# TaceoLabs/co-snarks

Measured on NVIDIA H100. Metric: co-Groth16 proofs/sec (BN254, 2^20 constraints); MSM Mscalar/s, higher is better.
Workload: dtype u32x8 (256-bit Montgomery, integer)

## Files before the change

### co_snarks_b200/csrc/cs_curve.cuh

```cuda
#pragma once
#include "cs_field.cuh"

namespace cs {

template <class P>
struct Fp2 {
  typedef Fp<P> F;
  static constexpr int N = 2 * P::N;
  F c0, c1;
  static CS_D Fp2 zero() { Fp2 r; r.c0 = F::zero(); r.c1 = F::zero(); return r; }
  static CS_D Fp2 one() { Fp2 r; r.c0 = F::one(); r.c1 = F::zero(); return r; }
  CS_D bool is_zero() const { return c0.is_zero() && c1.is_zero(); }
  CS_D bool operator==(const Fp2& b) const { return c0 == b.c0 && c1 == b.c1; }
  CS_D bool operator!=(const Fp2& b) const { return !(*this == b); }
  friend CS_D Fp2 operator+(const Fp2& a, const Fp2& b) { Fp2 r; r.c0 = a.c0 + b.c0; r.c1 = a.c1 + b.c1; return r; }
  friend CS_D Fp2 operator-(const Fp2& a, const Fp2& b) { Fp2 r; r.c0 = a.c0 - b.c0; r.c1 = a.c1 - b.c1; return r; }
  friend CS_D Fp2 operator*(const Fp2& a, const Fp2& b) { return mul_ool(a, b); }
  static CS_DN Fp2 mul_ool(Fp2 a, Fp2 b) {
    F v0 = F::mul_inline(a.c0, b.c0), v1 = F::mul_inline(a.c1, b.c1);
    F v2 = F::mul_inline(a.c0 + a.c1, b.c0 + b.c1);
    Fp2 r;
    r.c1 = v2 - v0 - v1;
    r.c0 = v0 - v1;
    return r;
  }
  CS_D Fp2 sqr() const { return sqr_ool(*this); }
  static CS_DN Fp2 sqr_ool(Fp2 a) {
    Fp2 r;
    F t = F::mul_inline(a.c0, a.c1);
    r.c0 = F::mul_inline(a.c0 + a.c1, a.c0 - a.c1);
    r.c1 = t + t;
    return r;
  }
  CS_D Fp2 neg() const { Fp2 r; r.c0 = c0.neg(); r.c1 = c1.neg(); return r; }
  CS_D Fp2 dbl() const { Fp2 r; r.c0 = c0.dbl(); r.c1 = c1.dbl(); return r; }
  CS_D Fp2 inverse() const {
    F n = (c0.sqr() + c1.sqr()).inverse();
    Fp2 r;
    r.c0 = c0 * n;
    r.c1 = (c1 * n).neg();
    return r;
  }
};

template <class P>
CS_D Fp<P> mul_sub(const Fp<P>& a, const Fp<P>& b, const Fp<P>& c, const Fp<P>& d) { return Fp<P>::dot2(a, b, c.neg(), d); }
template <class P>
CS_D Fp2<P> mul_sub(const Fp2<P>& a, const Fp2<P>& b, const Fp2<P>& c, const Fp2<P>& d) { return a * b - c * d; }

template <class F>
struct Affine {
  F x, y;
  CS_D bool is_inf() const { return x.is_zero() && y.is_zero(); }
  static CS_D Affine inf() { Affine r; r.x = F::zero(); r.y = F::zero(); return r; }
};

template <class F>
struct Xyzz {
  F x, y, zz, zzz;
  CS_D bool is_inf() const { return zz.is_zero(); }
  static CS_D Xyzz inf() {
    Xyzz r;
    r.x = F::zero(); r.y = F::zero(); r.zz = F::zero(); r.zzz = F::zero();
    return r;
  }
  static CS_D Xyzz from_affine(const Affine<F>& p) {
    if (p.is_inf()) return inf();
    Xyzz r;
    r.x = p.x; r.y = p.y; r.zz = F::one(); r.zzz = F::one();
    return r;
  }
};

template <class F>
CS_DN Xyzz<F> dbl_affine(const Affine<F>& p) {
  Xyzz<F> r;
  if (p.y.is_zero()) return Xyzz<F>::inf();
  F U = p.y.dbl();
  F V = U.sqr();
  F W = U * V;
  F S = p.x * V;
  F X2 = p.x.sqr();
  F M = X2.dbl() + X2;
  r.x = M.sqr() - S.dbl();
  r.y = mul_sub(M, S - r.x, W, p.y);
  r.zz = V;
  r.zzz = W;
  return r;
}

template <class F>
CS_DN Xyzz<F> dbl_xyzz(const Xyzz<F>& p) {
  if (p.is_inf() || p.y.is_zero()) return Xyzz<F>::inf();
  Xyzz<F> r;
  F U = p.y.dbl();
  F V = U.sqr();
  F W = U * V;
  F S = p.x * V;
  F X2 = p.x.sqr();
  F M = X2.dbl() + X2;
  r.x = M.sqr() - S.dbl();
  r.y = mul_sub(M, S - r.x, W, p.y);
  r.zz = V * p.zz;
  r.zzz = W * p.zzz;
  return r;
}

template <class F>
CS_D void madd(Xyzz<F>& acc, const Affine<F>& p_in, bool negate) {
  if (p_in.is_inf()) return;
  Affine<F> p = p_in;
  if (negate) p.y = p.y.neg();
  if (acc.is_inf()) {
    acc.x = p.x; acc.y = p.y; acc.zz = F::one(); acc.zzz = F::one();
    return;
  }
  F U2 = p.x * acc.zz;
  F S2 = p.y * acc.zzz;
  F Pp = U2 - acc.x;
  F R = S2 - acc.y;
  if (Pp.is_zero()) {
    if (R.is_zero()) acc = dbl_affine(p);
    else acc = Xyzz<F>::inf();
    return;
  }
  F PP = Pp.sqr();
  F PPP = Pp * PP;
  F Q = acc.x * PP;
  F X3 = R.sqr() - PPP - Q.dbl();
  acc.y = mul_sub(R, Q - X3, acc.y, PPP);
  acc.x = X3;
  acc.zz = acc.zz * PP;
  acc.zzz = acc.zzz * PPP;
}

template <class F>
CS_D void padd(Xyzz<F>& acc, const Xyzz<F>& q) {
  if (q.is_inf()) return;
  if (acc.is_inf()) { acc = q; return; }
  F U1 = acc.x * q.zz;
  F U2 = q.x * acc.zz;
  F S1 = acc.y * q.zzz;
  F S2 = q.y * acc.zzz;
  F Pp = U2 - U1;
  F R = S2 - S1;
  if (Pp.is_zero()) {
    if (R.is_zero()) acc = dbl_xyzz(acc);
    else acc = Xyzz<F>::inf();
    return;
  }
  F PP = Pp.sqr();
  F PPP = Pp * PP;
  F Q = U1 * PP;
  F X3 = R.sqr() - PPP - Q.dbl();
  acc.y = mul_sub(R, Q - X3, S1, PPP);
  acc.x = X3;
  acc.zz = acc.zz * q.zz * PP;
  acc.zzz = acc.zzz * q.zzz * PPP;
}

template <class P>
CS_D Fp<P> shfl_down(const Fp<P>& a, unsigned delta) {
  Fp<P> r;
#if defined(CS_EMU)
  cs::emu::shfl_bytes(&a, &r, sizeof(r), 1, delta);
  return r;
#endif
  CS_UNROLL
  for (int i = 0; i < P::N; i++) r.l[i] = __shfl_down_sync(0xffffffffu, a.l[i], delta);
  return r;
}
template <class P>
CS_D Fp2<P> shfl_down(const Fp2<P>& a, unsigned delta) {
  Fp2<P> r;
  r.c0 = shfl_down(a.c0, delta);
  r.c1 = shfl_down(a.c1, delta);
  return r;
}
template <class F>
CS_D Xyzz<F> shfl_down(const Xyzz<F>& p, unsigned delta) {
  Xyzz<F> r;
#if defined(CS_EMU)
  cs::emu::shfl_bytes(&p, &r, sizeof(r), 1, delta);
  return r;
#endif
  r.x = shfl_down(p.x, delta); r.y = shfl_down(p.y, delta);
  r.zz = shfl_down(p.zz, delta); r.zzz = shfl_down(p.zzz, delta);
  return r;
}

template <class F>
CS_DN Affine<F> to_affine(const Xyzz<F>& p) {
  if (p.is_inf()) return Affine<F>::inf();
  F zi = p.zzz.inverse();
  F zzi = (zi * p.zz).sqr();
  Affine<F> r;
  r.x = p.x * zzi;
  r.y = p.y * zi;
  return r;
}

}
```

### co_snarks_b200/csrc/cs_field.cuh

```cuda
#pragma once
#include "cs_prims.cuh"

namespace cs {

template <int N>
CS_D void mul_n(uint32_t* acc, const uint32_t* a, uint32_t bi) {
  CS_UNROLL
  for (int j = 0; j < N; j += 2) {
    acc[j] = mul_lo(a[j], bi);
    acc[j + 1] = mul_hi(a[j], bi);
  }
}

template <int N>
CS_D void cmad_n(uint32_t* acc, const uint32_t* a, uint32_t bi) {
  acc[0] = mad_lo_cc(a[0], bi, acc[0]);
  acc[1] = madc_hi_cc(a[0], bi, acc[1]);
  CS_UNROLL
  for (int j = 2; j < N; j += 2) {
    acc[j] = madc_lo_cc(a[j], bi, acc[j]);
    acc[j + 1] = madc_hi_cc(a[j], bi, acc[j + 1]);
  }
}

template <int N>
CS_D void madc_n_rshift(uint32_t* odd, const uint32_t* a, uint32_t bi) {
  CS_UNROLL
  for (int j = 0; j < N - 2; j += 2) {
    odd[j] = madc_lo_cc(a[j], bi, odd[j + 2]);
    odd[j + 1] = madc_hi_cc(a[j], bi, odd[j + 3]);
  }
  odd[N - 2] = madc_lo_cc(a[N - 2], bi, 0);
  odd[N - 1] = madc_hi(a[N - 2], bi, 0);
}

template <class P, bool FIRST>
CS_D void mad_n_redc(uint32_t* X, uint32_t* Y, const uint32_t* a, uint32_t bi) {
  constexpr int N = P::N;
  if (FIRST) {
    mul_n<N>(Y, a + 1, bi);
    mul_n<N>(X, a, bi);
  } else {
    X[0] = add_cc(X[0], Y[1]);
    madc_n_rshift<N>(Y, a + 1, bi);
    cmad_n<N>(X, a, bi);
    Y[N - 1] = addc(Y[N - 1], 0);
  }
  uint32_t mi = mul_lo(X[0], P::M0);
  uint32_t mod[N];
  CS_UNROLL
  for (int i = 0; i < N; i++) mod[i] = P::mod(i);
  cmad_n<N>(Y, mod + 1, mi);
  cmad_n<N>(X, mod, mi);
  Y[N - 1] = addc(Y[N - 1], 0);
}

template <class P>
struct Fp {
  static constexpr int N = P::N;
  uint32_t l[N];

  static CS_D Fp zero() { Fp r; CS_UNROLL for (int i = 0; i < N; i++) r.l[i] = 0; return r; }
  static CS_D Fp one() { Fp r; CS_UNROLL for (int i = 0; i < N; i++) r.l[i] = P::one(i); return r; }
  static CS_D Fp r2() { Fp r; CS_UNROLL for (int i = 0; i < N; i++) r.l[i] = P::r2(i); return r; }

  CS_D bool is_zero() const {
    uint32_t o = 0;
    CS_UNROLL
    for (int i = 0; i < N; i++) o |= l[i];
    return o == 0;
  }
  CS_D bool operator==(const Fp& b) const {
    uint32_t o = 0;
    CS_UNROLL
    for (int i = 0; i < N; i++) o |= l[i] ^ b.l[i];
    return o == 0;
  }
  CS_D bool operator!=(const Fp& b) const { return !(*this == b); }

  CS_D void final_sub() {
    uint32_t t[N];
    t[0] = sub_cc(l[0], P::mod(0));
    CS_UNROLL
    for (int i = 1; i < N; i++) t[i] = subc_cc(l[i], P::mod(i));
    uint32_t borrow = subc(0, 0);
    CS_UNROLL
    for (int i = 0; i < N; i++) l[i] = borrow ? l[i] : t[i];
  }

  friend CS_D Fp operator+(const Fp& a, const Fp& b) {
    Fp r;
    r.l[0] = add_cc(a.l[0], b.l[0]);
    CS_UNROLL
    for (int i = 1; i < N; i++) r.l[i] = addc_cc(a.l[i], b.l[i]);
    r.final_sub();
    return r;
  }
  friend CS_D Fp operator-(const Fp& a, const Fp& b) {
    Fp r;
    r.l[0] = sub_cc(a.l[0], b.l[0]);
    CS_UNROLL
    for (int i = 1; i < N; i++) r.l[i] = subc_cc(a.l[i], b.l[i]);
    uint32_t borrow = subc(0, 0);
    r.l[0] = add_cc(r.l[0], borrow & P::mod(0));
    CS_UNROLL
    for (int i = 1; i < N; i++) r.l[i] = addc_cc(r.l[i], borrow & P::mod(i));
    return r;
  }
  CS_D Fp neg() const { return is_zero() ? *this : (zero() - *this); }
  CS_D Fp dbl() const { return *this + *this; }

  friend CS_D Fp operator*(const Fp& a, const Fp& b) { return mul_ool(a, b); }
  static CS_DN Fp mul_ool(Fp a, Fp b) { return mul_inline(a, b); }
  static CS_D Fp mul_inline(const Fp& a, const Fp& b) {
    uint32_t even[N], odd[N];
    mad_n_redc<P, true>(even, odd, a.l, b.l[0]);
    mad_n_redc<P, false>(odd, even, a.l, b.l[1]);
    CS_UNROLL
    for (int i = 2; i < N; i += 2) {
      mad_n_redc<P, false>(even, odd, a.l, b.l[i]);
      mad_n_redc<P, false>(odd, even, a.l, b.l[i + 1]);
    }
    Fp r;
    r.l[0] = add_cc(even[0], odd[1]);
    CS_UNROLL
    for (int i = 1; i < N - 1; i++) r.l[i] = addc_cc(even[i], odd[i + 1]);
    r.l[N - 1] = addc(even[N - 1], 0);
    r.final_sub();
    return r;
  }
  CS_D Fp sqr() const { return sqr_ool(*this); }
  static CS_DN Fp sqr_ool(Fp a) {
    uint32_t c0 = 0, c1 = 0, c2 = 0;
    uint32_t m[N];
    Fp r;
    CS_UNROLL
    for (int k = 0; k < 2 * N - 1; k++) {
      uint32_t t0 = 0, t1 = 0, t2 = 0;
      CS_UNROLL
      for (int i = 0; i < N; i++) {
        int j = k - i;
        if (j > i && j < N) {
          t0 = mad_lo_cc(a.l[i], a.l[j], t0);
          t1 = madc_hi_cc(a.l[i], a.l[j], t1);
          t2 = addc(t2, 0);
        }
      }
      t2 = (t2 << 1) | (t1 >> 31);
      t1 = (t1 << 1) | (t0 >> 31);
      t0 = t0 << 1;
      c0 = add_cc(c0, t0);
      c1 = addc_cc(c1, t1);
      c2 = addc(c2, t2);
      if ((k & 1) == 0) {
        c0 = mad_lo_cc(a.l[k / 2], a.l[k / 2], c0);
        c1 = madc_hi_cc(a.l[k / 2], a.l[k / 2], c1);
        c2 = addc(c2, 0);
      }
      CS_UNROLL
      for (int i = 0; i < N; i++) {
        int j = k - i;
        if (i < k && i < N && j >= 0 && j < N && (k < N ? i < k : true)) {
          if (k < N || i >= k - N + 1) {
            c0 = mad_lo_cc(m[i], P::mod(j), c0);
            c1 = madc_hi_cc(m[i], P::mod(j), c1);
            c2 = addc(c2, 0);
          }
        }
      }
      if (k < N) {
        m[k] = mul_lo(c0, P::M0);
        c0 = mad_lo_cc(m[k], P::mod(0), c0);
        c1 = madc_hi_cc(m[k], P::mod(0), c1);
        c2 = addc(c2, 0);
      } else {
        r.l[k - N] = c0;
      }
      c0 = c1; c1 = c2; c2 = 0;
    }
    r.l[N - 1] = c0;
    r.final_sub();
    return r;
  }

  static CS_D Fp dot2(const Fp& a, const Fp& b, const Fp& c, const Fp& d) { return dot2_ool(a, b, c, d); }
  static CS_DN Fp dot2_ool(Fp a, Fp b, Fp c, Fp d) {
    uint32_t c0 = 0, c1 = 0, c2 = 0;
    uint32_t m[N];
    Fp r;
    CS_UNROLL
    for (int k = 0; k < 2 * N - 1; k++) {
      CS_UNROLL
      for (int i = 0; i < N; i++) {
        const int j = k - i;
        if (j >= 0 && j < N) {
          c0 = mad_lo_cc(a.l[i], b.l[j], c0);
          c1 = madc_hi_cc(a.l[i], b.l[j], c1);
          c2 = addc(c2, 0);
          c0 = mad_lo_cc(c.l[i], d.l[j], c0);
          c1 = madc_hi_cc(c.l[i], d.l[j], c1);
          c2 = addc(c2, 0);
        }
      }
      CS_UNROLL
      for (int i = 0; i < N; i++) {
        const int j = k - i;
        if (j >= 1 && j < N) {
          c0 = mad_lo_cc(m[i], P::mod(j), c0);
          c1 = madc_hi_cc(m[i], P::mod(j), c1);
          c2 = addc(c2, 0);
        }
      }
      if (k < N) {
        m[k] = mul_lo(c0, P::M0);
        c0 = mad_lo_cc(m[k], P::mod(0), c0);
        c1 = madc_hi_cc(m[k], P::mod(0), c1);
        c2 = addc(c2, 0);
      } else {
        r.l[k - N] = c0;
      }
      c0 = c1; c1 = c2; c2 = 0;
    }
    r.l[N - 1] = c0;
    r.final_sub();
    return r;
  }

  CS_D Fp to_mont() const { return (*this) * r2(); }
  CS_D Fp from_mont() const {
    Fp o = zero();
    o.l[0] = 1;
    return (*this) * o;
  }

  CS_D Fp inverse() const {
    Fp res = one();
    Fp base = *this;
    for (int i = 0; i < N; i++) {
      uint32_t e = P::mod(i);
      if (i == 0) e -= 2;
      for (int b = 0; b < 32; b++) {
        if ((e >> b) & 1) res = res * base;
        base = base.sqr();
      }
    }
    return res;
  }
};

}
```

### co_snarks_b200/csrc/cs_msm.cuh

```cuda
#pragma once
#include <stdlib.h>
#include "cs_common.cuh"
#include "cs_curve.cuh"

namespace cs {

constexpr unsigned MSM_SLICE_MAX = 64;
constexpr unsigned MSM_ORDER_BLOCK = 256;
constexpr unsigned MSM_RED_SEG = 4;
constexpr unsigned MSM_SIGN = 0x80000000u;

template <class FrP>
CS_GLOBAL void k_msm_digits(const uint32_t* __restrict__ scalars, uint32_t sstride, uint32_t n, int mont,
                            uint32_t c, uint32_t W, const uint32_t* __restrict__ infmask, uint32_t offset,
                            uint32_t* __restrict__ dig, uint32_t* __restrict__ count) {
  uint32_t i = blockIdx.x * blockDim.x + threadIdx.x;
  if (i >= n) return;
  if ((infmask[(offset + i) >> 5] >> ((offset + i) & 31)) & 1) {
    for (uint32_t w = 0; w < W; w++) dig[(size_t)w * n + i] = 0;
    return;
  }
  Fp<FrP> s;
  const uint4* src = reinterpret_cast<const uint4*>(scalars) + (size_t)i * sstride * (FrP::N / 4);
  CS_UNROLL
  for (int k = 0; k < FrP::N / 4; k++) {
    uint4 v = src[k];
    s.l[4 * k] = v.x; s.l[4 * k + 1] = v.y; s.l[4 * k + 2] = v.z; s.l[4 * k + 3] = v.w;
  }
  if (mont) s = s.from_mont();
  uint32_t lim[FrP::N + 1];
  CS_UNROLL
  for (int k = 0; k < FrP::N; k++) lim[k] = s.l[k];
  lim[FrP::N] = 0;
  const uint32_t half = 1u << (c - 1);
  const uint32_t mask = (1u << c) - 1;
  uint32_t carry = 0;
  for (uint32_t w = 0; w < W; w++) {
    uint32_t pos = w * c;
    uint32_t li = pos >> 5, sh = pos & 31;
    uint32_t lo = li < FrP::N ? lim[li] : 0;
    uint32_t hi = li + 1 < FrP::N ? lim[li + 1] : 0;
    uint32_t d = (__funnelshift_r(lo, hi, sh) & mask) + carry;
    uint32_t out;
    if (d > half) {
      out = ((1u << c) - d) | MSM_SIGN;
      carry = 1;
    } else {
      out = d;
      carry = 0;
    }
    dig[(size_t)w * n + i] = out;
    uint32_t b = out & ~MSM_SIGN;
    if (b) atomicAdd(&count[b], 1u);
  }
}

template <class F>
CS_GLOBAL void k_msm_infmask(const Affine<F>* __restrict__ table, uint32_t n, uint32_t* __restrict__ mask) {
  uint32_t wd = blockIdx.x * blockDim.x + threadIdx.x;
  if (wd * 32 >= n) return;
  uint32_t m = 0;
  for (uint32_t k = 0; k < 32 && wd * 32 + k < n; k++)
    if (table[wd * 32 + k].is_inf()) m |= 1u << k;
  mask[wd] = m;
}

constexpr unsigned MSM_SCAN_T = 1024;
constexpr unsigned MSM_SCAN_MAX_BLOCKS = 1024;
CS_D void msm_scan_terms(const uint32_t* __restrict__ count, uint32_t k, uint32_t nb1, uint32_t S, uint32_t* v) {
  uint32_t cnt = (k && k < nb1) ? count[k] : 0;
  uint32_t n0 = (cnt + S - 1) / S;
  uint32_t n1 = (n0 + S - 1) / S;
  v[0] = cnt; v[1] = n0; v[2] = n1; v[3] = (n1 + S - 1) / S;
}
static CS_GLOBAL void k_msm_scan1(const uint32_t* __restrict__ count, uint32_t nb1 , uint32_t S,
                                  uint32_t* __restrict__ start, uint32_t* __restrict__ sstart0,
                                  uint32_t* __restrict__ sstart1, uint32_t* __restrict__ sstart2, uint32_t* __restrict__ aux) {
  __shared__ uint32_t sm[4][32];
  const uint32_t t = threadIdx.x, lane = t & 31, wid = t >> 5, nwarp = blockDim.x >> 5;
  const uint32_t k = blockIdx.x * blockDim.x + t;
  uint32_t v[4], inc[4];
  msm_scan_terms(count, k, nb1, S, v);
  CS_UNROLL
  for (int q = 0; q < 4; q++) {
    uint32_t x = v[q];
    CS_UNROLL
    for (uint32_t d = 1; d < 32; d <<= 1) {
      uint32_t y = __shfl_up_sync(0xffffffffu, x, d);
      if (lane >= d) x += y;
    }
    inc[q] = x;
    if (lane == 31) sm[q][wid] = x;
  }
  __syncthreads();
  uint32_t w[4], x[4];
  CS_UNROLL
  for (int q = 0; q < 4; q++) {
    w[q] = (wid == 0 && lane < nwarp) ? sm[q][lane] : 0;
    x[q] = w[q];
    CS_UNROLL
    for (uint32_t d = 1; d < 32; d <<= 1) {
      uint32_t y = __shfl_up_sync(0xffffffffu, x[q], d);
      if (lane >= d) x[q] += y;
    }
  }
  __syncthreads();
  if (wid == 0 && lane < nwarp) {
    CS_UNROLL
    for (int q = 0; q < 4; q++) sm[q][lane] = x[q] - w[q];
    if (lane == nwarp - 1) {
      CS_UNROLL
      for (int q = 0; q < 4; q++) aux[blockIdx.x * 4 + q] = x[q];
    }
  }
  __syncthreads();
  if (k < nb1) {
    start[k] = sm[0][wid] + inc[0] - v[0];
    sstart0[k] = sm[1][wid] + inc[1] - v[1];
    sstart1[k] = sm[2][wid] + inc[2] - v[2];
    sstart2[k] = sm[3][wid] + inc[3] - v[3];
  }
}
static CS_GLOBAL void k_msm_scan2(const uint32_t* __restrict__ count, uint32_t nb1, uint32_t S,
                                  uint32_t* __restrict__ start, uint32_t* __restrict__ sstart0,
                                  uint32_t* __restrict__ sstart1, uint32_t* __restrict__ sstart2,
                                  const uint32_t* __restrict__ aux) {
  const uint32_t k = blockIdx.x * blockDim.x + threadIdx.x;
  if (k >= nb1) return;
  uint32_t off[4] = {0, 0, 0, 0};
  for (uint32_t b = 0; b < blockIdx.x; b++) {
    CS_UNROLL
    for (int q = 0; q < 4; q++) off[q] += aux[b * 4 + q];
  }
  uint32_t a = start[k] + off[0], b0 = sstart0[k] + off[1], b1 = sstart1[k] + off[2], b2 = sstart2[k] + off[3];
  start[k] = a; sstart0[k] = b0; sstart1[k] = b1; sstart2[k] = b2;
  if (k == nb1 - 1) {
    uint32_t v[4];
    msm_scan_terms(count, k, nb1, S, v);
    start[nb1] = a + v[0]; sstart0[nb1] = b0 + v[1]; sstart1[nb1] = b1 + v[2]; sstart2[nb1] = b2 + v[3];
  }
}

static CS_GLOBAL void k_msm_scatter(const uint32_t* __restrict__ dig, uint32_t n, uint32_t nbases,
                             uint32_t offset, const uint32_t* __restrict__ start,
                             uint32_t* __restrict__ cursor, uint32_t* __restrict__ sorted) {
  uint32_t i = blockIdx.x * blockDim.x + threadIdx.x;
  uint32_t w = blockIdx.y;
  if (i >= n) return;
  uint32_t d = dig[(size_t)w * n + i];
  uint32_t b = d & ~MSM_SIGN;
  if (!b) return;
  uint32_t pos = start[b] + atomicAdd(&cursor[b], 1u);
  sorted[pos] = (w * nbases + offset + i) | (d & MSM_SIGN);
}

CS_D uint32_t find_bucket(const uint32_t* __restrict__ arr, uint32_t nb1, uint32_t s) {
  uint32_t lo = 0, hi = nb1;
  while (hi - lo > 1) {
    uint32_t mid = (lo + hi) >> 1;
    if (arr[mid] <= s) lo = mid; else hi = mid;
  }
  return lo;
}

static CS_GLOBAL void k_msm_slice_hist(const uint32_t* __restrict__ count, const uint32_t* __restrict__ sstart0,
                                       uint32_t nb1, uint32_t S, uint32_t* __restrict__ slice_len,
                                       uint32_t* __restrict__ slice_bkt, uint32_t* __restrict__ block_hist) {
  __shared__ uint32_t h[MSM_SLICE_MAX + 1];
  for (uint32_t k = threadIdx.x; k <= MSM_SLICE_MAX; k += blockDim.x) h[k] = 0;
  __syncthreads();
  uint32_t s = blockIdx.x * blockDim.x + threadIdx.x;
  if (s < sstart0[nb1]) {
    uint32_t lo = 0, hi = nb1;
    while (hi - lo > 1) {
      uint32_t mid = (lo + hi) >> 1;
      if (sstart0[mid] <= s) lo = mid; else hi = mid;
    }
    uint32_t j = s - sstart0[lo];
    uint32_t len = count[lo] - j * S;
    if (len > S) len = S;
    slice_len[s] = len;
    slice_bkt[s] = lo;
    atomicAdd(&h[len], 1u);
  }
  __syncthreads();
  for (uint32_t k = threadIdx.x; k <= MSM_SLICE_MAX; k += blockDim.x)
    block_hist[(size_t)blockIdx.x * (MSM_SLICE_MAX + 1) + k] = h[k];
}

constexpr unsigned MSM_OFF_CHUNKS = 64;
static CS_GLOBAL void k_msm_slice_off1(const uint32_t* __restrict__ block_hist, uint32_t nblocks,
                                       uint32_t* __restrict__ chunk_sum) {
  uint32_t id = blockIdx.x * blockDim.x + threadIdx.x;
  if (id >= (MSM_SLICE_MAX + 1) * MSM_OFF_CHUNKS) return;
  uint32_t L = id / MSM_OFF_CHUNKS, ch = id % MSM_OFF_CHUNKS;
  uint32_t per = (nblocks + MSM_OFF_CHUNKS - 1) / MSM_OFF_CHUNKS;
  uint32_t lo = ch * per, hi = lo + per < nblocks ? lo + per : nblocks;
  uint32_t sum = 0;
  for (uint32_t b = lo; b < hi; b++) sum += block_hist[(size_t)b * (MSM_SLICE_MAX + 1) + L];
  chunk_sum[id] = sum;
}
static CS_GLOBAL void k_msm_slice_off2(uint32_t* __restrict__ chunk_sum, uint32_t* __restrict__ len_base) {
  uint32_t L = blockIdx.x * blockDim.x + threadIdx.x;
  if (L > MSM_SLICE_MAX) return;
  uint32_t run = 0;
  for (uint32_t c = 0; c < MSM_OFF_CHUNKS; c++) {
    uint32_t v = chunk_sum[L * MSM_OFF_CHUNKS + c];
    chunk_sum[L * MSM_OFF_CHUNKS + c] = run;
    run += v;
  }
  len_base[MSM_SLICE_MAX + 1 + L] = run;
}
static CS_GLOBAL void k_msm_slice_off3(uint32_t* __restrict__ block_hist, uint32_t nblocks,
                                       const uint32_t* __restrict__ chunk_sum, uint32_t* __restrict__ len_base) {
  uint32_t id = blockIdx.x * blockDim.x + threadIdx.x;
  if (id == 0) {
    uint32_t run = 0;
    for (int k = MSM_SLICE_MAX; k >= 0; k--) { len_base[k] = run; run += len_base[MSM_SLICE_MAX + 1 + k]; }
  }
  if (id >= (MSM_SLICE_MAX + 1) * MSM_OFF_CHUNKS) return;
  uint32_t L = id / MSM_OFF_CHUNKS, ch = id % MSM_OFF_CHUNKS;
  uint32_t per = (nblocks + MSM_OFF_CHUNKS - 1) / MSM_OFF_CHUNKS;
  uint32_t lo = ch * per, hi = lo + per < nblocks ? lo + per : nblocks;
  uint32_t run = chunk_sum[id];
  for (uint32_t b = lo; b < hi; b++) {
    uint32_t v = block_hist[(size_t)b * (MSM_SLICE_MAX + 1) + L];
    block_hist[(size_t)b * (MSM_SLICE_MAX + 1) + L] = run;
    run += v;
  }
}

static CS_GLOBAL void k_msm_slice_order(const uint32_t* __restrict__ slice_len, const uint32_t* __restrict__ slice_bkt,
                                        uint32_t nslices_max, const uint32_t* __restrict__ sstart0, uint32_t nb1,
                                        const uint32_t* __restrict__ block_off, const uint32_t* __restrict__ len_base,
                                        uint32_t* __restrict__ order, uint32_t* __restrict__ order_b) {
  __shared__ uint32_t h[MSM_SLICE_MAX + 1];
  for (uint32_t k = threadIdx.x; k <= MSM_SLICE_MAX; k += blockDim.x) h[k] = 0;
  __syncthreads();
  uint32_t s = blockIdx.x * blockDim.x + threadIdx.x;
  if (s < sstart0[nb1]) {
    uint32_t len = slice_len[s];
    uint32_t rank = atomicAdd(&h[len], 1u);
    uint32_t pos = len_base[len] + block_off[(size_t)blockIdx.x * (MSM_SLICE_MAX + 1) + len] + rank;
    order[pos] = s;
    order_b[pos] = slice_bkt[s];
  }
}

template <class F, int MINB>
CS_GLOBAL void __launch_bounds__(128, MINB) k_msm_accum0(const Affine<F>* __restrict__ table,
                                                         const uint32_t* __restrict__ sorted,
                                                         const uint32_t* __restrict__ count,
                                                         const uint32_t* __restrict__ start,
                                                         const uint32_t* __restrict__ sstart0, uint32_t nb1, uint32_t S,
                                                         const uint32_t* __restrict__ order,
                                                         const uint32_t* __restrict__ order_b,
                                                         Xyzz<F>* __restrict__ part0) {
  uint32_t t = blockIdx.x * blockDim.x + threadIdx.x;
  if (t >= sstart0[nb1]) return;
  uint32_t s = order[t];
  uint32_t b = order_b[t];
  uint32_t j = s - sstart0[b];
  uint32_t beg = start[b] + j * S;
  uint32_t end = start[b] + count[b];
  if (end > beg + S) end = beg + S;
  Xyzz<F> acc = Xyzz<F>::inf();
  uint32_t e = sorted[beg];
  Affine<F> p = table[e & ~MSM_SIGN];
  for (uint32_t k = beg; k < end; k++) {
    uint32_t e_cur = e;
    Affine<F> p_cur = p;
    if (k + 1 < end) {
      e = sorted[k + 1];
      p = table[e & ~MSM_SIGN];
    }
    madd(acc, p_cur, (e_cur & MSM_SIGN) != 0);
  }
  part0[s] = acc;
}

template <class F>
CS_GLOBAL void __launch_bounds__(128) k_msm_accum1(const Xyzz<F>* __restrict__ part0,
                                                   const uint32_t* __restrict__ sstart0,
                                                   const uint32_t* __restrict__ sstart1, uint32_t nb1, uint32_t S,
                                                   Xyzz<F>* __restrict__ part1) {
  uint32_t s = blockIdx.x * blockDim.x + threadIdx.x;
  if (s >= sstart1[nb1]) return;
  uint32_t b = find_bucket(sstart1, nb1, s);
  uint32_t j = s - sstart1[b];
  uint32_t beg = sstart0[b] + j * S;
  uint32_t end = sstart0[b + 1];
  if (end > beg + S) end = beg + S;
  Xyzz<F> acc = part0[beg];
  for (uint32_t k = beg + 1; k < end; k++) padd(acc, part0[k]);
  part1[s] = acc;
}

template <class F>
CS_GLOBAL void __launch_bounds__(128) k_msm_accum2(const Xyzz<F>* __restrict__ part1,
                                                   const uint32_t* __restrict__ sstart1, uint32_t nb1,
                                                   Xyzz<F>* __restrict__ bucket) {
  uint32_t b = blockIdx.x * blockDim.x + threadIdx.x;
  if (b >= nb1) return;
  uint32_t beg = sstart1[b], end = sstart1[b + 1];
  Xyzz<F> acc = Xyzz<F>::inf();
  if (beg < end) {
    acc = part1[beg];
    for (uint32_t k = beg + 1; k < end; k++) padd(acc, part1[k]);
  }
  bucket[b] = acc;
}

template <class F>
CS_GLOBAL void __launch_bounds__(128) k_msm_reduce_seg(const Xyzz<F>* __restrict__ bucket, uint32_t B,
                                                       uint32_t L, Xyzz<F>* __restrict__ red) {
  uint32_t t = blockIdx.x * blockDim.x + threadIdx.x;
  uint32_t lo = t * L;
  if (lo >= B) return;
  uint32_t hi = lo + L < B ? lo + L : B;
  Xyzz<F> acc = Xyzz<F>::inf(), tot = Xyzz<F>::inf();
  for (uint32_t b = hi; b > lo; b--) {
    padd(acc, bucket[b]);
    padd(tot, acc);
  }
  if (lo != 0 && !acc.is_inf()) {
    Xyzz<F> m = Xyzz<F>::inf();
    int top = 31 - __clz(lo);
    for (int bit = top; bit >= 0; bit--) {
      m = dbl_xyzz(m);
      if ((lo >> bit) & 1) padd(m, acc);
    }
    padd(tot, m);
  }
  red[t] = tot;
}

template <class F>
CS_GLOBAL void k_msm_final_sum(const Xyzz<F>* __restrict__ red, uint32_t cnt,
                                                      Xyzz<F>* __restrict__ out) {
  CS_DYN_SMEM(Xyzz<F>, sm);
  const uint32_t T = blockDim.x, t = threadIdx.x;
  Xyzz<F> acc = Xyzz<F>::inf();
  for (uint32_t k = blockIdx.x * T + t; k < cnt; k += gridDim.x * T) padd(acc, red[k]);
  sm[t] = acc;
  __syncthreads();
  for (uint32_t step = T >> 1; step > 0; step >>= 1) {
    if (t < step) {
      Xyzz<F> a = sm[t];
      padd(a, sm[t + step]);
      sm[t] = a;
    }
    __syncthreads();
  }
  if (t == 0) out[blockIdx.x] = sm[0];
}

constexpr int MSM_PRE_CHUNK = 8;
template <class F>
CS_GLOBAL void __launch_bounds__(128) k_msm_precompute(Affine<F>* __restrict__ table, uint32_t n,
                                                       uint32_t c, uint32_t W) {
  uint32_t i = blockIdx.x * blockDim.x + threadIdx.x;
  if (i >= n) return;
  Affine<F> p = table[i];
  if (p.is_inf()) {
    for (uint32_t w = 1; w < W; w++) table[(size_t)w * n + i] = Affine<F>::inf();
    return;
  }
  Xyzz<F> cur = Xyzz<F>::from_affine(p);
  uint32_t w = 1;
  while (w < W) {
    Xyzz<F> pts[MSM_PRE_CHUNK];
    F pre[MSM_PRE_CHUNK];
    int cnt = 0;
    bool degenerate = false;
    for (; cnt < MSM_PRE_CHUNK && w + cnt < W; cnt++) {
      for (uint32_t k = 0; k < c; k++) cur = dbl_xyzz(cur);
      pts[cnt] = cur;
      degenerate = degenerate || cur.is_inf();
    }
    Affine<F> last;
    if (degenerate) {
      for (int j = 0; j < cnt; j++) {
        last = to_affine(pts[j]);
        table[(size_t)(w + j) * n + i] = last;
      }
    } else {
      pre[0] = pts[0].zzz;
      for (int j = 1; j < cnt; j++) pre[j] = pre[j - 1] * pts[j].zzz;
      F inv = pre[cnt - 1].inverse();
      for (int j = cnt - 1; j >= 0; j--) {
        F zi = j ? inv * pre[j - 1] : inv;
        inv = inv * pts[j].zzz;
        F zzi = (zi * pts[j].zz).sqr();
        Affine<F> a;
        a.x = pts[j].x * zzi;
        a.y = pts[j].y * zi;
        table[(size_t)(w + j) * n + i] = a;
        if (j == cnt - 1) last = a;
      }
    }
    cur = Xyzz<F>::from_affine(last);
    w += cnt;
  }
}

template <class F, class FrP>
CS_GLOBAL void __launch_bounds__(128) k_fixed_base_mul(const Affine<F>* __restrict__ base,
                                                       const uint32_t* __restrict__ scalars, uint32_t n,
                                                       int mont, Affine<F>* __restrict__ out) {
  uint32_t i = blockIdx.x * blockDim.x + threadIdx.x;
  if (i >= n) return;
  Fp<FrP> s;
  const uint4* src = reinterpret_cast<const uint4*>(scalars) + (size_t)i * (FrP::N / 4);
  CS_UNROLL
  for (int k = 0; k < FrP::N / 4; k++) {
    uint4 v = src[k];
    s.l[4 * k] = v.x; s.l[4 * k + 1] = v.y; s.l[4 * k + 2] = v.z; s.l[4 * k + 3] = v.w;
  }
  if (mont) s = s.from_mont();
  uint32_t lim[FrP::N];
  CS_UNROLL
  for (int k = 0; k < FrP::N; k++) lim[k] = s.l[k];
  Affine<F> b = base[0];
  Xyzz<F> acc = Xyzz<F>::inf();
  for (int bit = FrP::N * 32 - 1; bit >= 0; bit--) {
    acc = dbl_xyzz(acc);
    if ((lim[bit >> 5] >> (bit & 31)) & 1) madd(acc, b, false);
  }
  out[i] = to_affine(acc);
}

struct MsmShape {
  uint32_t c, W, B;
};

static inline MsmShape msm_shape(uint32_t scalar_bits, uint32_t c) {
  MsmShape s;
  s.c = c;
  s.W = (scalar_bits + 1 + c - 1) / c;
  s.B = 1u << (c - 1);
  return s;
}

static inline uint32_t msm_auto_window(size_t n, uint32_t scalar_bits) {
  int lg = 0;
  while ((1ull << (lg + 1)) <= n) lg++;
  int c = lg >= 15 ? 16 : lg - 4;
  if (c < 4) c = 4;
  while (c < 16) {
    const uint32_t W = (scalar_bits + 1 + c - 1) / c;
    const uint32_t top = scalar_bits + 1 - (W - 1) * c;
    if (2 * top >= (uint32_t)c) break;
    c++;
  }
  return (uint32_t)c;
}
static inline uint32_t msm_slice(const MsmShape& sh) {
  const char* e = getenv("CS_MSM_SLICE");
  if (e && atoi(e) == 64) return 64u;
  if (e && atoi(e) == 32) return 32u;
  return sh.c >= 18 ? 64u : 32u;
}

constexpr int MSM_NSTAGE = 5;
struct MsmWorkspace {
  DevBuf dig, sorted, meta, part0, part1, part2, bucket, red, scal, result, order;
  void* h_result = nullptr;
  size_t h_result_cap = 0;
  bool profile = false;
  cudaEvent_t ev[MSM_NSTAGE + 1] = {};
  cudaEvent_t sorted_ev = nullptr;
  bool sorted_ev_made = false, sorted_once = false;
  cudaEvent_t acc_in = nullptr, acc_out = nullptr;
  int mark(int i, cudaStream_t st) {
    if (!profile) return 0;
    if (!ev[i]) CS_CUDA(cudaEventCreateWithFlags(&ev[i], 0));
    CS_CUDA(cudaEventRecord(ev[i], st));
    return 0;
  }
  void release() {
    for (int i = 0; i <= MSM_NSTAGE; i++) {
      if (ev[i]) cudaEventDestroy(ev[i]);
      ev[i] = nullptr;
    }
    if (sorted_ev_made) cudaEventDestroy(sorted_ev);
    if (acc_in) cudaEventDestroy(acc_in);
    if (acc_out) cudaEventDestroy(acc_out);
    acc_in = acc_out = nullptr;
    sorted_ev = nullptr;
    sorted_ev_made = sorted_once = false;
    dig.release(); sorted.release(); meta.release(); part0.release(); part1.release(); part2.release();
    bucket.release(); red.release(); scal.release(); result.release(); order.release();
    if (h_result) cudaFreeHost(h_result);
    h_result = nullptr;
    h_result_cap = 0;
  }
};

template <class F>
int msm_accum0_f52(const Affine<F>* table, const uint32_t* sorted, const uint32_t* count, const uint32_t* start,
                   const uint32_t* sstart0, uint32_t nb1, uint32_t S, const uint32_t* order, const uint32_t* order_b,
                   Xyzz<F>* part0, uint32_t max_s0, cudaStream_t st);

template <class F, class FrP>
int msm_enqueue(MsmWorkspace& ws, const Affine<F>* table, const uint32_t* infmask, uint32_t nbases, MsmShape sh,
                uint32_t offset,
                const uint32_t* d_scalars, uint32_t sstride, uint32_t n, int mont, cudaStream_t st,
                MsmWorkspace* sort_from = nullptr, bool table_m260 = false, cudaStream_t st_acc = nullptr) {
  const uint32_t nb1 = sh.B + 1;
  const size_t nent = (size_t)sh.W * n;
  if (nent >= (1ull << 31) || (size_t)sh.W * nbases >= (1ull << 31))
    return fail(-3, "msm: W*n = %zu exceeds 2^31 entries", nent);
  const uint32_t S = msm_slice(sh);
  const size_t max_s0 = nent / S + nb1;
  const size_t max_s1 = max_s0 / S + nb1;
  const size_t max_s2 = max_s1 / S + nb1;
  MsmWorkspace& so = sort_from ? *sort_from : ws;
  const size_t meta_words = 2 * (size_t)nb1 + 4 * ((size_t)nb1 + 1) + 4 * MSM_SCAN_MAX_BLOCKS;
  if (!sort_from) {
    CS_TRY(ws.dig.reserve(nent * 4));
    CS_TRY(ws.sorted.reserve(nent * 4));
    CS_TRY(ws.meta.reserve(meta_words * 4));
  }
  CS_TRY(ws.part0.reserve(max_s0 * sizeof(Xyzz<F>)));
  CS_TRY(ws.part1.reserve(max_s1 * sizeof(Xyzz<F>)));
  CS_TRY(ws.part2.reserve(max_s2 * sizeof(Xyzz<F>)));
  CS_TRY(ws.bucket.reserve((size_t)nb1 * sizeof(Xyzz<F>)));
  const uint32_t L = sh.B < MSM_RED_SEG ? sh.B : MSM_RED_SEG;
  const uint32_t nseg = (sh.B + L - 1) / L;
  const uint32_t fs_threads = sizeof(Xyzz<F>) > 128 ? 128 : 256;
  const uint32_t fs_blocks = nseg > 4 * fs_threads ? (nseg + fs_threads - 1) / fs_threads : 1;
  CS_TRY(ws.red.reserve(((size_t)nseg + fs_blocks) * sizeof(Xyzz<F>)));
  CS_TRY(ws.result.reserve(sizeof(Xyzz<F>)));
  const uint32_t ob = ceil_div(max_s0, MSM_ORDER_BLOCK);
  const size_t order_words = 4 * max_s0 + (size_t)ob * (MSM_SLICE_MAX + 1) + 2 * (MSM_SLICE_MAX + 1) +
                             (size_t)(MSM_SLICE_MAX + 1) * MSM_OFF_CHUNKS;
  if (!sort_from) CS_TRY(ws.order.reserve(order_words * 4));
  if (ws.h_result_cap < sizeof(Xyzz<F>)) {
    if (ws.h_result) cudaFreeHost(ws.h_result);
    CS_CUDA(cudaMallocHost(&ws.h_result, sizeof(Xyzz<F>)));
    ws.h_result_cap = sizeof(Xyzz<F>);
  }
  uint32_t* slice_len = so.order.as<uint32_t>();
  uint32_t* slice_bkt = slice_len + max_s0;
  uint32_t* order = slice_bkt + max_s0;
  uint32_t* order_b = order + max_s0;
  uint32_t* block_hist = order_b + max_s0;
  uint32_t* len_base = block_hist + (size_t)ob * (MSM_SLICE_MAX + 1);
  uint32_t* chunk_sum = len_base + 2 * (MSM_SLICE_MAX + 1);
  uint32_t* count = so.meta.as<uint32_t>();
  uint32_t* cursor = count + nb1;
  uint32_t* start = cursor + nb1;
  uint32_t* sstart0 = start + nb1 + 1;
  uint32_t* sstart1 = sstart0 + nb1 + 1;
  uint32_t* sstart2 = sstart1 + nb1 + 1;
  if (sort_from) {
    if (!sort_from->sorted_once) return fail(-1, "msm: the workspace to share a sort with has not been enqueued");
    CS_TRY(ws.mark(0, st));
    CS_CUDA(cudaStreamWaitEvent(st, sort_from->sorted_ev, 0));
    CS_TRY(ws.mark(1, st));
  } else {
    CS_TRY(ws.mark(0, st));
    CS_CUDA(cudaMemsetAsync(count, 0, 2 * (size_t)nb1 * 4, st));
    CS_LAUNCH(k_msm_digits<FrP>, ceil_div(n, 256), 256, 0, st, d_scalars, sstride, n, mont, sh.c, sh.W, infmask, offset,
              ws.dig.as<uint32_t>(), count);
    CS_TRY(ws.mark(1, st));
    {
      const uint32_t sb = ceil_div(nb1, MSM_SCAN_T);
      if (sb > MSM_SCAN_MAX_BLOCKS) return fail(-3, "msm: %u buckets exceed the scan's limit", sh.B);
      uint32_t* aux = sstart2 + nb1 + 1;
      CS_LAUNCH_SYNC(k_msm_scan1, sb, MSM_SCAN_T, 0, st, count, nb1, S, start, sstart0, sstart1, sstart2, aux);
      CS_LAUNCH(k_msm_scan2, sb, MSM_SCAN_T, 0, st, count, nb1, S, start, sstart0, sstart1, sstart2, aux);
    }
    CS_LAUNCH(k_msm_scatter, dim3(ceil_div(n, 256), sh.W), 256, 0, st, ws.dig.as<uint32_t>(), n, nbases,
              offset, start, cursor, ws.sorted.as<uint32_t>());
    CS_LAUNCH_SYNC(k_msm_slice_hist, ob, MSM_ORDER_BLOCK, 0, st, count, sstart0, nb1, S, slice_len, slice_bkt, block_hist);
    {
      const uint32_t nt = (MSM_SLICE_MAX + 1) * MSM_OFF_CHUNKS;
      CS_LAUNCH(k_msm_slice_off1, ceil_div(nt, 128), 128, 0, st, block_hist, ob, chunk_sum);
      CS_LAUNCH(k_msm_slice_off2, 1, 128, 0, st, chunk_sum, len_base);
      CS_LAUNCH(k_msm_slice_off3, ceil_div(nt, 128), 128, 0, st, block_hist, ob, chunk_sum, len_base);
    }
    CS_LAUNCH_SYNC(k_msm_slice_order, ob, MSM_ORDER_BLOCK, 0, st, slice_len, slice_bkt, (uint32_t)max_s0, sstart0, nb1,
                   block_hist, len_base, order, order_b);
    if (!ws.sorted_ev_made) {
      CS_CUDA(cudaEventCreateWithFlags(&ws.sorted_ev, cudaEventDisableTiming));
      ws.sorted_ev_made = true;
    }
    CS_CUDA(cudaEventRecord(ws.sorted_ev, st));
    ws.sorted_once = true;
  }
  CS_TRY(ws.mark(2, st));
  cudaStream_t st_main = st;
  if (st_acc) {
    if (!ws.acc_in) {
      CS_CUDA(cudaEventCreateWithFlags(&ws.acc_in, cudaEventDisableTiming));
      CS_CUDA(cudaEventCreateWithFlags(&ws.acc_out, cudaEventDisableTiming));
    }
    CS_CUDA(cudaEventRecord(ws.acc_in, st));
    CS_CUDA(cudaStreamWaitEvent(st_acc, ws.acc_in, 0));
    st = st_acc;
  }
  {
    static int minb_env = -1;
    if (minb_env < 0) { const char* e = getenv("CS_ACCUM0_MINB"); minb_env = e ? atoi(e) : 0; }
    const int minb = minb_env ? minb_env : 4;
    if (table_m260) {
      CS_TRY((msm_accum0_f52<F>(table, so.sorted.as<uint32_t>(), count, start, sstart0, nb1, S, order, order_b,
                                ws.part0.as<Xyzz<F>>(), (uint32_t)max_s0, st)));
    } else {
#define CS_ACC0(M)                                                                                              \
  CS_LAUNCH(k_msm_accum0<F COMMA M>, ceil_div(max_s0, 128), 128, 0, st, table, so.sorted.as<uint32_t>(), count, \
            start, sstart0, nb1, S, order, order_b, ws.part0.as<Xyzz<F>>())
    switch (minb) {
      case 2: CS_ACC0(2); break;
      case 3: CS_ACC0(3); break;
      case 5: CS_ACC0(5); break;
      case 6: CS_ACC0(6); break;
      default: CS_ACC0(4); break;
    }
#undef CS_ACC0
    }
  }
  if (st_acc) {
    CS_CUDA(cudaEventRecord(ws.acc_out, st_acc));
    st = st_main;
    CS_CUDA(cudaStreamWaitEvent(st, ws.acc_out, 0));
  }
  CS_TRY(ws.mark(3, st));
  CS_LAUNCH(k_msm_accum1<F>, ceil_div(max_s1, 128), 128, 0, st, ws.part0.as<Xyzz<F>>(), sstart0, sstart1,
            nb1, S, ws.part1.as<Xyzz<F>>());
  CS_LAUNCH(k_msm_accum1<F>, ceil_div(max_s2, 128), 128, 0, st, ws.part1.as<Xyzz<F>>(), sstart1, sstart2,
            nb1, S, ws.part2.as<Xyzz<F>>());
  CS_LAUNCH(k_msm_accum2<F>, ceil_div(nb1, 128), 128, 0, st, ws.part2.as<Xyzz<F>>(), sstart2, nb1,
            ws.bucket.as<Xyzz<F>>());
  CS_TRY(ws.mark(4, st));
  CS_LAUNCH(k_msm_reduce_seg<F>, ceil_div(nseg, 128), 128, 0, st, ws.bucket.as<Xyzz<F>>(), sh.B, L,
            ws.red.as<Xyzz<F>>());
  if (fs_blocks > 1) {
    Xyzz<F>* stage = ws.red.as<Xyzz<F>>() + nseg;
    CS_LAUNCH_SYNC(k_msm_final_sum<F>, fs_blocks, fs_threads, fs_threads * sizeof(Xyzz<F>), st, ws.red.as<Xyzz<F>>(), nseg,
                   stage);
    CS_LAUNCH_SYNC(k_msm_final_sum<F>, 1, fs_threads, fs_threads * sizeof(Xyzz<F>), st, stage, fs_blocks,
                   ws.result.as<Xyzz<F>>());
  } else {
    CS_LAUNCH_SYNC(k_msm_final_sum<F>, 1, fs_threads, fs_threads * sizeof(Xyzz<F>), st, ws.red.as<Xyzz<F>>(), nseg,
                   ws.result.as<Xyzz<F>>());
  }
  CS_TRY(ws.mark(5, st));
  CS_CUDA(cudaMemcpyAsync(ws.h_result, ws.result.p, sizeof(Xyzz<F>), cudaMemcpyDeviceToHost, st));
  CS_CUDA(cudaGetLastError());
  return 0;
}

}
```

### co_snarks_b200/csrc/cs_prims.cuh

```cuda
#pragma once
#include <stdint.h>

#if defined(CS_EMU)
#include "cs_emu.h"
#define CS_D inline
#define CS_DN __attribute__((noinline))
#define CS_HD inline
#define CS_GLOBAL
#define CS_UNROLL
#else
#include <cuda_runtime.h>
#define CS_D __device__ __forceinline__
#define CS_DN __device__ __noinline__
#define CS_HD __host__ __device__ __forceinline__
#define CS_GLOBAL __global__
#define CS_UNROLL _Pragma("unroll")
#endif

namespace cs {

#if defined(CS_EMU)
inline uint32_t& cf_() { static thread_local uint32_t cf = 0; return cf; }
inline uint32_t add_cc(uint32_t a, uint32_t b) { uint64_t s = (uint64_t)a + b; cf_() = (uint32_t)(s >> 32); return (uint32_t)s; }
inline uint32_t addc_cc(uint32_t a, uint32_t b) { uint64_t s = (uint64_t)a + b + cf_(); cf_() = (uint32_t)(s >> 32); return (uint32_t)s; }
inline uint32_t addc(uint32_t a, uint32_t b) { return (uint32_t)((uint64_t)a + b + cf_()); }
inline uint32_t sub_cc(uint32_t a, uint32_t b) { uint64_t d = (uint64_t)a - b; cf_() = (uint32_t)((d >> 32) & 1); return (uint32_t)d; }
inline uint32_t subc_cc(uint32_t a, uint32_t b) { uint64_t d = (uint64_t)a - b - cf_(); cf_() = (uint32_t)((d >> 32) & 1); return (uint32_t)d; }
inline uint32_t subc(uint32_t a, uint32_t b) { return (uint32_t)((uint64_t)a - b - cf_()); }
inline uint32_t mul_lo(uint32_t a, uint32_t b) { return (uint32_t)((uint64_t)a * b); }
inline uint32_t mul_hi(uint32_t a, uint32_t b) { return (uint32_t)(((uint64_t)a * b) >> 32); }
inline uint32_t mad_lo_cc(uint32_t a, uint32_t b, uint32_t c) { return add_cc(mul_lo(a, b), c); }
inline uint32_t madc_lo_cc(uint32_t a, uint32_t b, uint32_t c) { return addc_cc(mul_lo(a, b), c); }
inline uint32_t mad_hi_cc(uint32_t a, uint32_t b, uint32_t c) { return add_cc(mul_hi(a, b), c); }
inline uint32_t madc_hi_cc(uint32_t a, uint32_t b, uint32_t c) { return addc_cc(mul_hi(a, b), c); }
inline uint32_t madc_hi(uint32_t a, uint32_t b, uint32_t c) { return addc(mul_hi(a, b), c); }
#else
CS_D uint32_t add_cc(uint32_t a, uint32_t b) { uint32_t r; asm volatile("add.cc.u32 %0, %1, %2;" : "=r"(r) : "r"(a), "r"(b)); return r; }
CS_D uint32_t addc_cc(uint32_t a, uint32_t b) { uint32_t r; asm volatile("addc.cc.u32 %0, %1, %2;" : "=r"(r) : "r"(a), "r"(b)); return r; }
CS_D uint32_t addc(uint32_t a, uint32_t b) { uint32_t r; asm volatile("addc.u32 %0, %1, %2;" : "=r"(r) : "r"(a), "r"(b)); return r; }
CS_D uint32_t sub_cc(uint32_t a, uint32_t b) { uint32_t r; asm volatile("sub.cc.u32 %0, %1, %2;" : "=r"(r) : "r"(a), "r"(b)); return r; }
CS_D uint32_t subc_cc(uint32_t a, uint32_t b) { uint32_t r; asm volatile("subc.cc.u32 %0, %1, %2;" : "=r"(r) : "r"(a), "r"(b)); return r; }
CS_D uint32_t subc(uint32_t a, uint32_t b) { uint32_t r; asm volatile("subc.u32 %0, %1, %2;" : "=r"(r) : "r"(a), "r"(b)); return r; }
CS_D uint32_t mul_lo(uint32_t a, uint32_t b) { uint32_t r; asm volatile("mul.lo.u32 %0, %1, %2;" : "=r"(r) : "r"(a), "r"(b)); return r; }
CS_D uint32_t mul_hi(uint32_t a, uint32_t b) { uint32_t r; asm volatile("mul.hi.u32 %0, %1, %2;" : "=r"(r) : "r"(a), "r"(b)); return r; }
CS_D uint32_t mad_lo_cc(uint32_t a, uint32_t b, uint32_t c) { uint32_t r; asm volatile("mad.lo.cc.u32 %0, %1, %2, %3;" : "=r"(r) : "r"(a), "r"(b), "r"(c)); return r; }
CS_D uint32_t madc_lo_cc(uint32_t a, uint32_t b, uint32_t c) { uint32_t r; asm volatile("madc.lo.cc.u32 %0, %1, %2, %3;" : "=r"(r) : "r"(a), "r"(b), "r"(c)); return r; }
CS_D uint32_t mad_hi_cc(uint32_t a, uint32_t b, uint32_t c) { uint32_t r; asm volatile("mad.hi.cc.u32 %0, %1, %2, %3;" : "=r"(r) : "r"(a), "r"(b), "r"(c)); return r; }
CS_D uint32_t madc_hi_cc(uint32_t a, uint32_t b, uint32_t c) { uint32_t r; asm volatile("madc.hi.cc.u32 %0, %1, %2, %3;" : "=r"(r) : "r"(a), "r"(b), "r"(c)); return r; }
CS_D uint32_t madc_hi(uint32_t a, uint32_t b, uint32_t c) { uint32_t r; asm volatile("madc.hi.u32 %0, %1, %2, %3;" : "=r"(r) : "r"(a), "r"(b), "r"(c)); return r; }
#endif

}
```

Before: 42.27.

## Use lazy-reduction wide products for Fp2 mul/mul_sub and prefetch G2 bucket points

Result: faster. 44.89, median of 6 (+6.2%).

```diff
diff --git a/co_snarks_b200/csrc/cs_curve.cuh b/co_snarks_b200/csrc/cs_curve.cuh
--- a/co_snarks_b200/csrc/cs_curve.cuh
+++ b/co_snarks_b200/csrc/cs_curve.cuh
@@ -17,11 +17,44 @@
   friend CS_D Fp2 operator-(const Fp2& a, const Fp2& b) { Fp2 r; r.c0 = a.c0 - b.c0; r.c1 = a.c1 - b.c1; return r; }
   friend CS_D Fp2 operator*(const Fp2& a, const Fp2& b) { return mul_ool(a, b); }
   static CS_DN Fp2 mul_ool(Fp2 a, Fp2 b) {
-    F v0 = F::mul_inline(a.c0, b.c0), v1 = F::mul_inline(a.c1, b.c1);
-    F v2 = F::mul_inline(a.c0 + a.c1, b.c0 + b.c1);
-    Fp2 r;
-    r.c1 = v2 - v0 - v1;
-    r.c0 = v0 - v1;
+    constexpr int W = 2 * P::N;
+    uint32_t v0[W], v1[W], v2[W];
+    F::mul_wide(v0, a.c0, b.c0);
+    F::mul_wide(v1, a.c1, b.c1);
+    F::mul_wide(v2, F::add_unreduced(a.c0, a.c1), F::add_unreduced(b.c0, b.c1));
+    sub_n<W>(v2, v0);
+    sub_n<W>(v2, v1);
+    add_mod_sq<P, 1>(v0);
+    sub_n<W>(v0, v1);
+    Fp2 r;
+    r.c0 = F::redc(v0);
+    r.c1 = F::redc(v2);
+    return r;
+  }
+  static CS_DN Fp2 mul_sub_ool(Fp2 a, Fp2 b, Fp2 c, Fp2 d) {
+    constexpr int W = 2 * P::N;
+    uint32_t t0[W], t1[W], t[W];
+    CS_UNROLL
+    for (int i = 0; i < W; i++) t0[i] = t1[i] = mod_sq<P, 2>(i);
+    F::mul_wide(t, a.c0, b.c0);
+    add_n<W>(t0, t);
+    sub_n<W>(t1, t);
+    F::mul_wide(t, a.c1, b.c1);
+    sub_n<W>(t0, t);
+    sub_n<W>(t1, t);
+    F::mul_wide(t, F::add_unreduced(a.c0, a.c1), F::add_unreduced(b.c0, b.c1));
+    add_n<W>(t1, t);
+    F::mul_wide(t, c.c0, d.c0);
+    sub_n<W>(t0, t);
+    add_n<W>(t1, t);
+    F::mul_wide(t, c.c1, d.c1);
+    add_n<W>(t0, t);
+    add_n<W>(t1, t);
+    F::mul_wide(t, F::add_unreduced(c.c0, c.c1), F::add_unreduced(d.c0, d.c1));
+    sub_n<W>(t1, t);
+    Fp2 r;
+    r.c0 = F::redc(t0);
+    r.c1 = F::redc(t1);
     return r;
   }
   CS_D Fp2 sqr() const { return sqr_ool(*this); }
@@ -46,7 +79,9 @@
 template <class P>
 CS_D Fp<P> mul_sub(const Fp<P>& a, const Fp<P>& b, const Fp<P>& c, const Fp<P>& d) { return Fp<P>::dot2(a, b, c.neg(), d); }
 template <class P>
-CS_D Fp2<P> mul_sub(const Fp2<P>& a, const Fp2<P>& b, const Fp2<P>& c, const Fp2<P>& d) { return a * b - c * d; }
+CS_D Fp2<P> mul_sub(const Fp2<P>& a, const Fp2<P>& b, const Fp2<P>& c, const Fp2<P>& d) {
+  return Fp2<P>::mul_sub_ool(a, b, c, d);
+}
 
 template <class F>
 struct Affine {
diff --git a/co_snarks_b200/csrc/cs_field.cuh b/co_snarks_b200/csrc/cs_field.cuh
--- a/co_snarks_b200/csrc/cs_field.cuh
+++ b/co_snarks_b200/csrc/cs_field.cuh
@@ -53,6 +53,73 @@
   cmad_n<N>(Y, mod + 1, mi);
   cmad_n<N>(X, mod, mi);
   Y[N - 1] = addc(Y[N - 1], 0);
+}
+
+template <int N>
+CS_D void mad_n(uint32_t* X, uint32_t* Y, const uint32_t* a, uint32_t bi) {
+  X[0] = add_cc(X[0], Y[1]);
+  madc_n_rshift<N>(Y, a + 1, bi);
+  cmad_n<N>(X, a, bi);
+  Y[N - 1] = addc(Y[N - 1], 0);
+}
+template <class P>
+CS_D void redc_row(uint32_t* X, uint32_t* Y, const uint32_t* mod) {
+  constexpr int N = P::N;
+  const uint32_t m = mul_lo(X[0] + Y[1], P::M0);
+  X[0] = add_cc(X[0], Y[1]);
+  madc_n_rshift<N>(Y, mod + 1, m);
+  cmad_n<N>(X, mod, m);
+  Y[N - 1] = addc(Y[N - 1], 0);
+}
+
+template <int M>
+CS_D void add_n(uint32_t* r, const uint32_t* a) {
+  r[0] = add_cc(r[0], a[0]);
+  CS_UNROLL
+  for (int i = 1; i < M - 1; i++) r[i] = addc_cc(r[i], a[i]);
+  r[M - 1] = addc(r[M - 1], a[M - 1]);
+}
+template <int M>
+CS_D void sub_n(uint32_t* r, const uint32_t* a) {
+  r[0] = sub_cc(r[0], a[0]);
+  CS_UNROLL
+  for (int i = 1; i < M - 1; i++) r[i] = subc_cc(r[i], a[i]);
+  r[M - 1] = subc(r[M - 1], a[M - 1]);
+}
+
+template <class P, int K>
+struct ModSq {
+  uint32_t v[2 * P::N];
+  CS_HD constexpr ModSq() : v{} {
+    for (int i = 0; i < P::N; i++) {
+      uint64_t carry = 0;
+      for (int j = 0; j < P::N; j++) {
+        const uint64_t s = (uint64_t)P::mod(i) * P::mod(j) + v[i + j] + carry;
+        v[i + j] = (uint32_t)s;
+        carry = s >> 32;
+      }
+      v[i + P::N] = (uint32_t)carry;
+    }
+    uint64_t carry = 0;
+    for (int k = 0; k < 2 * P::N; k++) {
+      const uint64_t s = (uint64_t)v[k] * K + carry;
+      v[k] = (uint32_t)s;
+      carry = s >> 32;
+    }
+  }
+};
+template <class P, int K>
+CS_HD constexpr uint32_t mod_sq(int k) {
+  constexpr ModSq<P, K> t;
+  return t.v[k];
+}
+template <class P, int K>
+CS_D void add_mod_sq(uint32_t* r) {
+  constexpr int M = 2 * P::N;
+  r[0] = add_cc(r[0], mod_sq<P, K>(0));
+  CS_UNROLL
+  for (int i = 1; i < M - 1; i++) r[i] = addc_cc(r[i], mod_sq<P, K>(i));
+  r[M - 1] = addc(r[M - 1], mod_sq<P, K>(M - 1));
 }
 
 template <class P>
@@ -226,6 +293,59 @@
     return r;
   }
 
+  static CS_D Fp add_unreduced(const Fp& a, const Fp& b) {
+    Fp r;
+    r.l[0] = add_cc(a.l[0], b.l[0]);
+    CS_UNROLL
+    for (int i = 1; i < N - 1; i++) r.l[i] = addc_cc(a.l[i], b.l[i]);
+    r.l[N - 1] = addc(a.l[N - 1], b.l[N - 1]);
+    return r;
+  }
+  static CS_D void mul_wide(uint32_t* t, const Fp& a, const Fp& b) {
+    uint32_t even[N], odd[N];
+    mul_n<N>(odd, a.l + 1, b.l[0]);
+    mul_n<N>(even, a.l, b.l[0]);
+    t[0] = even[0];
+    CS_UNROLL
+    for (int i = 1; i < N; i += 2) {
+      mad_n<N>(odd, even, a.l, b.l[i]);
+      t[i] = odd[0];
+      if (i + 1 < N) {
+        mad_n<N>(even, odd, a.l, b.l[i + 1]);
+        t[i + 1] = even[0];
+      }
+    }
+    t[N] = add_cc(even[0], odd[1]);
+    CS_UNROLL
+    for (int k = 1; k < N - 1; k++) t[N + k] = addc_cc(even[k], odd[k + 1]);
+    t[2 * N - 1] = addc(even[N - 1], 0);
+  }
+  static CS_D Fp redc(const uint32_t* t) {
+    uint32_t even[N], odd[N], mod[N];
+    CS_UNROLL
+    for (int i = 0; i < N; i++) { even[i] = t[i]; mod[i] = P::mod(i); }
+    const uint32_t m = mul_lo(even[0], P::M0);
+    mul_n<N>(odd, mod + 1, m);
+    cmad_n<N>(even, mod, m);
+    odd[N - 1] = addc(odd[N - 1], 0);
+    CS_UNROLL
+    for (int i = 1; i < N; i += 2) {
+      redc_row<P>(odd, even, mod);
+      if (i + 1 < N) redc_row<P>(even, odd, mod);
+    }
+    Fp r;
+    r.l[0] = add_cc(even[0], odd[1]);
+    CS_UNROLL
+    for (int k = 1; k < N - 1; k++) r.l[k] = addc_cc(even[k], odd[k + 1]);
+    r.l[N - 1] = addc(even[N - 1], 0);
+    r.l[0] = add_cc(r.l[0], t[N]);
+    CS_UNROLL
+    for (int k = 1; k < N - 1; k++) r.l[k] = addc_cc(r.l[k], t[N + k]);
+    r.l[N - 1] = addc(r.l[N - 1], t[2 * N - 1]);
+    r.final_sub();
+    return r;
+  }
+
   CS_D Fp to_mont() const { return (*this) * r2(); }
   CS_D Fp from_mont() const {
     Fp o = zero();
diff --git a/co_snarks_b200/csrc/cs_msm.cuh b/co_snarks_b200/csrc/cs_msm.cuh
--- a/co_snarks_b200/csrc/cs_msm.cuh
+++ b/co_snarks_b200/csrc/cs_msm.cuh
@@ -266,6 +266,18 @@
   if (end > beg + S) end = beg + S;
   Xyzz<F> acc = Xyzz<F>::inf();
   uint32_t e = sorted[beg];
+  if constexpr (sizeof(Affine<F>) > 64) {
+    for (uint32_t k = beg; k < end; k++) {
+      const uint32_t e_cur = e;
+      if (k + 1 < end) {
+        e = sorted[k + 1];
+        prefetch_l1(table + (e & ~MSM_SIGN));
+      }
+      madd(acc, table[e_cur & ~MSM_SIGN], (e_cur & MSM_SIGN) != 0);
+    }
+    part0[s] = acc;
+    return;
+  }
   Affine<F> p = table[e & ~MSM_SIGN];
   for (uint32_t k = beg; k < end; k++) {
     uint32_t e_cur = e;
@@ -604,7 +616,7 @@
   {
     static int minb_env = -1;
     if (minb_env < 0) { const char* e = getenv("CS_ACCUM0_MINB"); minb_env = e ? atoi(e) : 0; }
-    const int minb = minb_env ? minb_env : 4;
+    const int minb = minb_env ? minb_env : (sizeof(Affine<F>) > 64 ? 2 : 4);
     if (table_m260) {
       CS_TRY((msm_accum0_f52<F>(table, so.sorted.as<uint32_t>(), count, start, sstart0, nb1, S, order, order_b,
                                 ws.part0.as<Xyzz<F>>(), (uint32_t)max_s0, st)));
diff --git a/co_snarks_b200/csrc/cs_prims.cuh b/co_snarks_b200/csrc/cs_prims.cuh
--- a/co_snarks_b200/csrc/cs_prims.cuh
+++ b/co_snarks_b200/csrc/cs_prims.cuh
@@ -34,6 +34,7 @@
 inline uint32_t mad_hi_cc(uint32_t a, uint32_t b, uint32_t c) { return add_cc(mul_hi(a, b), c); }
 inline uint32_t madc_hi_cc(uint32_t a, uint32_t b, uint32_t c) { return addc_cc(mul_hi(a, b), c); }
 inline uint32_t madc_hi(uint32_t a, uint32_t b, uint32_t c) { return addc(mul_hi(a, b), c); }
+inline void prefetch_l1(const void*) {}
 #else
 CS_D uint32_t add_cc(uint32_t a, uint32_t b) { uint32_t r; asm volatile("add.cc.u32 %0, %1, %2;" : "=r"(r) : "r"(a), "r"(b)); return r; }
 CS_D uint32_t addc_cc(uint32_t a, uint32_t b) { uint32_t r; asm volatile("addc.cc.u32 %0, %1, %2;" : "=r"(r) : "r"(a), "r"(b)); return r; }
@@ -48,6 +49,7 @@
 CS_D uint32_t mad_hi_cc(uint32_t a, uint32_t b, uint32_t c) { uint32_t r; asm volatile("mad.hi.cc.u32 %0, %1, %2, %3;" : "=r"(r) : "r"(a), "r"(b), "r"(c)); return r; }
 CS_D uint32_t madc_hi_cc(uint32_t a, uint32_t b, uint32_t c) { uint32_t r; asm volatile("madc.hi.cc.u32 %0, %1, %2, %3;" : "=r"(r) : "r"(a), "r"(b), "r"(c)); return r; }
 CS_D uint32_t madc_hi(uint32_t a, uint32_t b, uint32_t c) { uint32_t r; asm volatile("madc.hi.u32 %0, %1, %2, %3;" : "=r"(r) : "r"(a), "r"(b), "r"(c)); return r; }
+CS_D void prefetch_l1(const void* p) { asm volatile("prefetch.global.L1 [%0];" ::"l"(p)); }
 #endif
 
 }
```
